# j04n-f/Encrypt-zkVM

Measured on AMD Instinct MI355X. Metric: STARK prove: trace-steps/sec at 2^20 steps; achieved HBM GB/s vs 8 TB/s peak, higher is better.
Workload: dtype f128

## Files before the change

encrypt-zkvm_amd/csrc/diag.hip:

```cpp
#include <hip/hip_runtime.h>
#include <string.h>

#include <algorithm>
#include <mutex>
#include <string>
#include <vector>

#include "blake3.hpp"
#include "host_pool.hpp"
#include "prover_internal.hpp"

using namespace zk;

namespace zk {
__global__ void k_field_op(int op, const fe *a, const fe *b, fe *out, size_t count, const fe_ws *ws, const fe_w2 *w2) {
    size_t t = blockIdx.x * (size_t)blockDim.x + threadIdx.x;
    if (t >= count) return;
    fe x = a[t], y = b[t];
    fe r;
    const size_t w0 = t & ~(size_t)63, mir = count - 1 - t;
    switch (op) {
    case 11: r = fe_mul_uniform(x, load_fe_ws(ws, (int)w0)); break;
    case 12: r = fe_mul_wsv(x, ws[t]); break;
    case 13: {
// ... 762 lines not shown
    for (int k = 0; k < W; k++) {
        TS.mode[k] = modes[k];
        if (modes[k] == CoeffSrc::ZERO) TS.plane[k] = nullptr;
        if (modes[k] != CoeffSrc::PLAIN) TS.lagr = p->polys + (size_t)W * n;
    }
    const Planes b = planes(p, ext);
    return with_kx(ext, [&](auto kx) -> int {
        constexpr int KX = decltype(kx)::value;
        typedef Chal<KX> X;
        const typename X::T zz = X::make(zv), zzg = X::make(zgv);
        ood_eval(p->st, TS, W, p->cpolys, ccols, log_n, zz, zzg, b.ood_tab, b.partials, p->ood);
        std::vector<fe> raw((size_t)KX * ood_out_values(TS, W, ccols)), hv((size_t)KX * (2 * W + ccols));
        ZK_TRY(p.down(raw.data(), p->ood, raw.size()));
        ood_fold_sources(KX, W, ccols, TS, wv, raw.data(), hv.data());
        memcpy(ood_out, hv.data(), hv.size() * sizeof(fe));
        DeepConsts<KX> D;
        memset(&D, 0, sizeof D);
        for (int k = 0; k < W; k++) D.alpha_t[k] = X::make(at[k]);
        for (int k = 0; k < C; k++) D.alpha_c[k] = X::make(ac[k]);
        D.z = zz, D.zg = zzg;
        deep_source_weight(D, TS, wv);
        ZK_CHECK_HIP(hipMemcpy(b.deep_consts, &D, sizeof D, hipMemcpyHostToDevice));
        const fe *Dk = deep_poly(p->st, TS, p->cpolys, C, log_n, b.deep_consts, zz, zzg, b.dscratch);
        ZK_TRY(p.down(deep_out, Dk, (size_t)KX * n));
        ZK_CHECK_HIP(hipMemsetAsync(p->flag, 0, 4, p->st));
        ZK_CHECK_HIP(hipMemsetAsync(p->ctmp, 0, (size_t)KX * n * 16, p->st));
        for (int j = 0; j < KX; j++)
            boundary_poly_add(p->st, TS, wv, log_n, K[j], cv, p->dscratch, p->ctmp + (size_t)j * n, p->flag);
        ZK_TRY(p.down(col0_out, p->ctmp, (size_t)KX * n));
        return p.down(flag_out, p->flag, 1);
    });
}

extern "C" int zk_diag_fri_layer(int device, const uint8_t *layer, size_t L, int ext, int fold, int lb, size_t wstride,
                                 const uint8_t *alpha, uint8_t *root_out, uint8_t *next_out) {
    fe2 av;
    const size_t N = L * wstride;
    const bool ok = layer && alpha && root_out && next_out && (ext == 1 || ext == 2) &&
                    (fold == 2 || fold == 4 || fold == 8 || fold == 16) && L && !(L & (L - 1)) && wstride &&
                    !(wstride & (wstride - 1)) && (L >= 4 * (size_t)fold || L == (size_t)fold) && N >= 128 &&
                    N <= ((size_t)1 << 22) && lb >= 0 && ((size_t)1 << lb) <= L / fold;
    if (!ok || !diag_read_fe(alpha, ext, &av))
        ZK_FAIL(ZK_ERR_INVALID_ARG, "zk_diag_fri_layer: L and wstride powers of two, 128 <= L wstride <= 2^22, fold 2 .. 16, "
                                    "at least 4 rows or the single row of an overfolded last layer, 2^lb <= L / fold, "
                                    "alpha canonical");
    DiagProver p;
    ZK_TRY(p.open(device, N / 8, 8, true, ext));
    const Planes b = planes(p, ext);
    const size_t rows = L / fold;
    uint8_t *leaves = p->fri_dig, *nodes = leaves + 32 * rows;
    ZK_CHECK_HIP(hipMemsetAsync(leaves, 0xA5, 64 * rows + 64, p->st));
    ZK_TRY(p.up(b.deep, layer, (size_t)ext * L));
    ZK_TRY(with_kx(ext, [&](auto kx) -> int {
        const auto F = fold_consts<decltype(kx)::value>(av, (uint32_t)fold);
        ZK_CHECK_HIP(hipMemcpy(b.fold_consts, &F, sizeof F, hipMemcpyHostToDevice));
        return ZK_OK;
    }));
    commit_fri_layer(p->st, ext, b.deep, L, fold, leaves, nodes, lb);
    fri_fold_launch(p->st, ext, b.deep, L, fold, b.fold_consts, p.pl->TN, wstride, b.fri, lb);
    ZK_TRY(p.down(root_out, nodes + 32, 32));
    return p.down(next_out, b.fri, (size_t)ext * rows);
}

constexpr size_t ZK_DIAG_MERKLE_GUARD = 4096;
extern "C" int zk_diag_merkle(int device, const uint8_t *leaves, size_t nl, int l3_min_log, uint32_t pf_blocks,
                              uint32_t block_p, uint8_t *nodes_out, uint8_t *guard_out, uint8_t *leaves_out,
                              const uint64_t *positions, size_t k, uint8_t *proof_out, size_t *proof_len) {
    if (!leaves || !nodes_out || !guard_out || !leaves_out || nl < 2 || (nl & (nl - 1)) || nl > ((size_t)1 << 24))
        ZK_FAIL(ZK_ERR_INVALID_ARG, "zk_diag_merkle: nl a power of two in [2, 2^24]");
    if (l3_min_log < 2 || l3_min_log > 62 || pf_blocks < 1 || pf_blocks > (1u << 20) || block_p < 1 || block_p > 512 ||
        (block_p & (block_p - 1)))
        ZK_FAIL(ZK_ERR_INVALID_ARG, "zk_diag_merkle: l3_min_log in [2, 62], pf_blocks in [1, 2^20], block_p a power of two "
                                    "in [1, 512]");
    if (positions && !proof_len) ZK_FAIL(ZK_ERR_INVALID_ARG, "zk_diag_merkle: positions without proof_len");
    std::vector<uint64_t> pos;
    if (positions) ZK_TRY(query_positions(positions, k, nl, pos));
    const size_t G = ZK_DIAG_MERKLE_GUARD, heap = 32 * nl;
    DiagBuf buf;
    ZK_TRY(buf.alloc(device, 2 * G + 2 * heap));
    uint8_t *d_nodes = buf.d + G, *d_leaves = buf.d + 2 * G + heap;
    ZK_CHECK_HIP(hipMemset(buf.d, 0xA5, 2 * G + heap));
    ZK_CHECK_HIP(hipMemcpy(d_leaves, leaves, heap, hipMemcpyHostToDevice));
    merkle_tree_cfg(nullptr, d_leaves, nl, d_nodes, MerkleCfg{l3_min_log, pf_blocks, block_p});
    ZK_CHECK_HIP(hipGetLastError());
    ZK_CHECK_HIP(hipMemcpy(nodes_out, d_nodes, heap, hipMemcpyDeviceToHost));
    ZK_CHECK_HIP(hipMemcpy(guard_out, buf.d, G, hipMemcpyDeviceToHost));
    ZK_CHECK_HIP(hipMemcpy(guard_out + G, d_nodes + heap, G, hipMemcpyDeviceToHost));
    ZK_CHECK_HIP(hipMemcpy(leaves_out, d_leaves, heap, hipMemcpyDeviceToHost));
    if (positions) ZK_TRY(batch_proof_bytes(nl, pos, d_leaves, d_nodes, proof_out, proof_len));
    return ZK_OK;
}

constexpr size_t ZK_DIAG_CE_GUARD = 4096;
extern "C" int zk_diag_ce_layout(int device, const uint8_t *in, size_t n, int ext, int to_natural, uint32_t max_blocks,
// ... 186 lines not shown
```

encrypt-zkvm_amd/csrc/fri_small.hpp:

```cpp
#pragma once
#include "f128.hpp"

namespace zk {
template <int F>
__device__ __forceinline__ void idft_small(fe v[F], const fe *zinv) {
    constexpr int LOGF = F == 2 ? 1 : F == 4 ? 2 : F == 8 ? 3 : 4;
    fe w[F];
#pragma unroll
    for (int k = 0; k < F; k++) {
        int r = 0;
#pragma unroll
        for (int b = 0; b < LOGF; b++) r |= ((k >> b) & 1) << (LOGF - 1 - b);
        w[r] = v[k];
    }
#pragma unroll
    for (int len = 2; len <= F; len <<= 1) {
#pragma unroll
        for (int start = 0; start < F; start += len) {
#pragma unroll
            for (int j = 0; j < len / 2; j++) {
                const fe u = w[start + j];
                const fe t = j == 0 ? w[start + j + len / 2] : fe_mul(w[start + j + len / 2], zinv[j * (F / len)]);
                w[start + j] = fe_add(u, t);
                w[start + j + len / 2] = fe_sub(u, t);
            }
        }
    }
#pragma unroll
    for (int k = 0; k < F; k++) v[k] = w[k];
}

}
```

encrypt-zkvm_amd/csrc/kernels.hip:

```cpp
#include <hip/hip_runtime.h>
#include <bitset>
#include <mutex>
#include <stdlib.h>
#include <string.h>

#include "blake3.hpp"
#include "fri_small.hpp"
#include "rescue_consts.hpp"
#include "zk_internal.hpp"

namespace zk {

#define ZK_LAUNCH_CHECK() (void)hipGetLastError()

__device__ __forceinline__ fe ld_fe(const fe *p) { return *p; }
__device__ __forceinline__ void st_fe(fe *p, fe v) { *p = v; }

template <class T>
__device__ __forceinline__ T pow_split(const T *lo, const T *hi, size_t t) {
    return ChalOf<T>::mul(lo[t & 2047], hi[t >> 11]);
}

#ifndef ZK_NTT_THREADS
#define ZK_NTT_THREADS 1024
#endif
#ifndef ZK_NTT_TILE
#define ZK_NTT_TILE 4096
#endif
#ifndef ZK_NTT_WAVES
#define ZK_NTT_WAVES 8
#endif
constexpr int NTT_THREADS = ZK_NTT_THREADS;

#ifndef ZK_NTT_LAZY
#define ZK_NTT_LAZY 1
#endif
#ifndef ZK_NTT_J0
#define ZK_NTT_J0 1
#endif
#ifndef ZK_NTT_SWZ
// ... 995 lines not shown
        v[0] = w.x;
        v[1] = w.y;
        v[2] = w.z;
        v[3] = w.w;
    }
#pragma unroll
    for (int e = 0; e < 4; e++) {
        const size_t i = i0 + e;
        out[i] = i == n - 1 ? nc.last[k] : fe{(uint64_t)v[e], 0};
    }
}

void expand_narrow(hipStream_t st, const uint8_t *src, const NarrowCols &nc, size_t n, fe *trace) {
    if (!nc.count) return;
    hipLaunchKernelGGL(k_expand_narrow, dim3(cdiv(n / 4, 256), nc.count), dim3(256), 0, st, src, nc, n, trace);
}

void commit_rows_coset_major(hipStream_t st, const fe *base, int ncols, int log_n, int log_b, uint8_t *leaves,
                             uint8_t *nodes) {
    const size_t N = (size_t)1 << (log_n + log_b);
    hash_rows_cosets(st, base, ncols, log_n, log_b, 0, log_b, leaves);
    merkle_tree(st, leaves, N, nodes);
}

__device__ __forceinline__ size_t fri_at(FriLayout f, size_t i) {
    return ((i & (((size_t)1 << f.lb) - 1)) << f.lcn) + (i >> f.lb);
}
FriLayout fri_layout(size_t L, int lb) {
    int lg = 0;
    while (((size_t)1 << lg) < L) lg++;
    return FriLayout{lb, lg - lb};
}

template <int KX>
__global__ void __launch_bounds__(256) k_hash_fri_rows(const fe *layer, size_t L, int fold, FriLayout f, uint8_t *leaves) {
    const size_t rows = L / fold;
    for (size_t r = blockIdx.x * (size_t)blockDim.x + threadIdx.x; r < rows; r += (size_t)gridDim.x * blockDim.x) {
        uint32_t h[8];
        b3::hash_elements(KX * fold, [&](int t) { return layer[(size_t)(t % KX) * L + fri_at(f, r + (size_t)(t / KX) * rows)]; }, h);
        store_digest(leaves + 32 * r, h);
    }
}

void commit_fri_layer(hipStream_t st, int KX, const fe *layer, size_t L, int fold, uint8_t *leaves, uint8_t *nodes, int lb) {
    const size_t rows = L / fold;
    const FriLayout f = fri_layout(L, lb);
    const dim3 grid(cdiv(rows, 256));
    if (KX == 1)
        ZK_PROF(st, "hash_fri_rows", 16.0 * L + 32.0 * rows, hipLaunchKernelGGL(k_hash_fri_rows<1>, grid, dim3(256), 0, st, layer, L, fold, f, leaves));
    else
        ZK_PROF(st, "hash_fri_rows_ext", 32.0 * L + 32.0 * rows, hipLaunchKernelGGL(k_hash_fri_rows<2>, grid, dim3(256), 0, st, layer, L, fold, f, leaves));
    if (rows == 1) (void)hipMemsetAsync(nodes + 32, 0, 32, st);
    merkle_tree(st, leaves, rows, nodes);
}

constexpr unsigned MERKLE_PF_BLOCKS = 2048;
__device__ __forceinline__ void merge_half3(const uint4 c[8], uint8_t *nodes, size_t cnt, size_t t, int half,
                                            uint32_t g[8]) {
    uint32_t l[8], r[8], h0[8], h1[8];
    auto dig = [&](int k, uint32_t d[8]) {
        const uint4 a = c[2 * k], b = c[2 * k + 1];
        d[0] = a.x; d[1] = a.y; d[2] = a.z; d[3] = a.w;
        d[4] = b.x; d[5] = b.y; d[6] = b.z; d[7] = b.w;
    };
    const size_t c0 = 4 * t + 2 * half;
    dig(0, l);
    dig(1, r);
    b3::merge(l, r, h0);
    store_digest(nodes + 32 * (cnt + c0), h0);
    dig(2, l);
    dig(3, r);
    b3::merge(l, r, h1);
    store_digest(nodes + 32 * (cnt + c0 + 1), h1);
    b3::merge(h0, h1, g);
    store_digest(nodes + 32 * (cnt / 2 + 2 * t + half), g);
}
#ifndef ZK_MERKLE_WAVES
#define ZK_MERKLE_WAVES 4
#endif
__global__ void __launch_bounds__(256, ZK_MERKLE_WAVES) k_merge_level3_pf(const uint8_t *src, uint8_t *nodes, size_t cnt) {
    const size_t q = cnt / 4, stride = (size_t)gridDim.x * blockDim.x;
    size_t t = blockIdx.x * (size_t)blockDim.x + threadIdx.x;
    const uint4 *s4 = reinterpret_cast<const uint4 *>(src);
    uint4 cur[8], nxt[8];
// ... 766 lines not shown

__global__ void __launch_bounds__(256) k_poly_degrees(const fe *polys, size_t len, DegReport *rep) {
    __shared__ unsigned long long sh_top[4];
    const int k = blockIdx.y;
    const fe *c = polys + (size_t)k * len;
    unsigned long long top = 0;
    for (size_t j = blockIdx.x * (size_t)blockDim.x + threadIdx.x; j < len; j += (size_t)gridDim.x * blockDim.x)
        if (!fe_is_zero(c[j])) top = j + 1;
    for (int d = 32; d > 0; d >>= 1) {
        const unsigned long long o = __shfl_xor(top, d, 64);
        top = o > top ? o : top;
    }
    if ((threadIdx.x & 63) == 0) sh_top[threadIdx.x >> 6] = top;
    __syncthreads();
    if (threadIdx.x == 0) {
        for (int w = 1; w < 4; w++) top = sh_top[w] > top ? sh_top[w] : top;
        if (top) {
            atomicMax(&rep->top[k], top - 1);
            atomicOr(&rep->nonzero, 1u << k);
        }
    }
}

void poly_degrees(hipStream_t st, const fe *polys, size_t len, int count, DegReport *rep) {
    unsigned blocks = cdiv(len, 256);
    if (blocks > 1024) blocks = 1024;
    ZK_PROF(st, "poly_degrees", 16.0 * count * (double)len,
            hipLaunchKernelGGL(k_poly_degrees, dim3(blocks, count), dim3(256), 0, st, polys, len, rep));
}

struct CrossWs {
    fe_ws w1, w2, w3, inv3n, k7[7];
};
__global__ void __launch_bounds__(256) k_comp_cross(CrossMap m, const fe *wi_lo, const fe *wi_hi,
                                                    const fe *i3_lo, const fe *i3_hi, fe scale, CrossWs cw,
                                                    int ncols, fe *polys, unsigned *nonzero) {
    for (size_t kl = blockIdx.x * (size_t)blockDim.x + threadIdx.x; kl < m.kcount; kl += (size_t)gridDim.x * blockDim.x) {
        const size_t k1 = m.k0 + kl;
        fe w = pow_split(wi_lo, wi_hi, k1);
        fe d[8];
        fe wr = fe_one();
#pragma unroll
        for (int r = 0; r < 8; r++) {
            if (r == 7 && m.derive7) {
                acc192 a7 = acc192_zero();
#pragma unroll
                for (int j = 0; j < 7; j++) acc192_madd_uniform(a7, d[j], cw.k7[j]);
                d[7] = acc192_reduce(a7);
                break;
            }
            fe v = m.c[r][kl];
            d[r] = r ? fe_mul(v, wr) : v;
            wr = fe_mul(wr, w);
        }
        fe e0 = d[0], e1 = d[4], e2 = d[2], e3 = d[6], e4 = d[1], e5 = d[5], e6 = d[3], e7 = d[7];
        fe t0 = fe_add(e0, e1), t1 = fe_sub(e0, e1), t2 = fe_add(e2, e3), t3 = fe_sub(e2, e3);
        fe t4 = fe_add(e4, e5), t5 = fe_sub(e4, e5), t6 = fe_add(e6, e7), t7 = fe_sub(e6, e7);
        t3 = fe_mul_uniform(t3, cw.w2);
        t7 = fe_mul_uniform(t7, cw.w2);
        fe u0 = fe_add(t0, t2), u2 = fe_sub(t0, t2), u1 = fe_add(t1, t3), u3 = fe_sub(t1, t3);
        fe u4 = fe_add(t4, t6), u6 = fe_sub(t4, t6), u5 = fe_add(t5, t7), u7 = fe_sub(t5, t7);
        u5 = fe_mul_uniform(u5, cw.w1);
        u6 = fe_mul_uniform(u6, cw.w2);
        u7 = fe_mul_uniform(u7, cw.w3);
        fe bk[8] = {fe_add(u0, u4), fe_add(u1, u5), fe_add(u2, u6), fe_add(u3, u7),
                    fe_sub(u0, u4), fe_sub(u1, u5), fe_sub(u2, u6), fe_sub(u3, u7)};
        fe s = fe_mul(scale, pow_split(i3_lo, i3_hi, k1));
        unsigned nz = 0;
#pragma unroll
        for (int k2 = 0; k2 < 8; k2++) {
            fe a = fe_mul(bk[k2], s);
            if (k2 < ncols) polys[(size_t)k2 * m.pstride + kl] = a;
            else nz |= !fe_is_zero(a);
            s = fe_mul_uniform(s, cw.inv3n);
        }
        if (nz) atomicOr(nonzero, 1u);
    }
}

void comp_cross_mapped(hipStream_t st, const CrossMap &m, const NttTables &T8n, const PowTable &inv3, fe scale,
                       fe w8inv, fe inv3n, int ncols, fe *polys, unsigned *nonzero_flag) {
    unsigned blocks = cdiv(m.kcount, 256);
    if (blocks > 65536) blocks = 65536;
    CrossWs cw;
    const fe w2 = fe_mul(w8inv, w8inv);
    cw.w1 = make_fe_ws(w8inv), cw.w2 = make_fe_ws(w2), cw.w3 = make_fe_ws(fe_mul(w2, w8inv));
    cw.inv3n = make_fe_ws(inv3n);
    for (int j = 0; j < 7; j++) cw.k7[j] = make_fe_ws(m.k7[j]);
    ZK_PROF(st, "comp_cross", (128.0 + 16.0 * ncols) * m.kcount, hipLaunchKernelGGL(k_comp_cross, dim3(blocks), dim3(256), 0, st, m, T8n.inv_lo,
                                                 T8n.inv_hi, inv3.lo, inv3.hi, scale, cw, ncols, polys,
                                                 nonzero_flag));
}

template <bool COEFFS>
__global__ void __launch_bounds__(256) k_cross_degrees(DegCrossMap m, const fe *wi_lo, const fe *wi_hi,
                                                       const fe *i3_lo, const fe *i3_hi, fe scale, CrossWs cw,
                                                       DegReport *rep) {
    __shared__ unsigned long long sh_top[4];
    const int k = blockIdx.y;
    const fe *c = m.c + (size_t)k * m.cstride;
    unsigned long long top = 0;
    for (size_t kl = blockIdx.x * (size_t)blockDim.x + threadIdx.x; kl < m.kcount; kl += (size_t)gridDim.x * blockDim.x) {
        const size_t k1 = m.k0 + kl;
        fe w = pow_split(wi_lo, wi_hi, k1);
        fe d[8];
        fe wr = fe_one();
#pragma unroll
        for (int r = 0; r < 8; r++) {
            fe v = c[m.off[r] + kl];
            d[r] = r ? fe_mul(v, wr) : v;
            wr = fe_mul(wr, w);
        }
        fe e0 = d[0], e1 = d[4], e2 = d[2], e3 = d[6], e4 = d[1], e5 = d[5], e6 = d[3], e7 = d[7];
        fe t0 = fe_add(e0, e1), t1 = fe_sub(e0, e1), t2 = fe_add(e2, e3), t3 = fe_sub(e2, e3);
        fe t4 = fe_add(e4, e5), t5 = fe_sub(e4, e5), t6 = fe_add(e6, e7), t7 = fe_sub(e6, e7);
        t3 = fe_mul_uniform(t3, cw.w2);
        t7 = fe_mul_uniform(t7, cw.w2);
        fe u0 = fe_add(t0, t2), u2 = fe_sub(t0, t2), u1 = fe_add(t1, t3), u3 = fe_sub(t1, t3);
        fe u4 = fe_add(t4, t6), u6 = fe_sub(t4, t6), u5 = fe_add(t5, t7), u7 = fe_sub(t5, t7);
        u5 = fe_mul_uniform(u5, cw.w1);
// ... 55 lines not shown
        ZK_PROF(st, "cross_degrees", 128.0 * m.count * (double)m.kcount,
                hipLaunchKernelGGL(k_cross_degrees<false>, grid, dim3(256), 0, st, m, T8n.inv_lo, T8n.inv_hi, inv3.lo,
                                   inv3.hi, scale, cw, rep));
}

constexpr int OOD_GROUP = 7;

template <int KX>
__global__ void k_ood_tables(typename Chal<KX>::T z, typename Chal<KX>::T zg, uint64_t chunk, int nw,
                             typename Chal<KX>::T *tab) {
    typedef typename Chal<KX>::T T;
    const int t = blockIdx.x * blockDim.x + threadIdx.x;
    if (t >= 128 + 2 * nw) return;
    T x;
    uint64_t e;
    if (t < 128) {
        x = t < 64 ? z : zg;
        e = t & 63;
    } else {
        const int u = t - 128;
        x = u < nw ? z : zg;
        e = chunk * (uint64_t)(u < nw ? u : u - nw);
    }
    tab[t] = Chal<KX>::exp(x, e);
}

struct OodPolys {
    static constexpr int MAXP = CoeffSrc::MAXC + 16 + 1;
    int count, count2;
    uint32_t zero;
    const fe *poly[MAXP];
    uint8_t rz[MAXP], rg[MAXP];
};
template <int KX, int E>
__global__ void __launch_bounds__(256) k_ood_eval(OodPolys L, int W, int np, size_t n, const typename Chal<KX>::T *tab,
                                                  int nw, int w0, int w1, fe *partials) {
    typedef Chal<KX> X;
    typedef typename X::T T;
    const int gw = w0 + (int)((blockIdx.x * blockDim.x + threadIdx.x) >> 6);
    const int lane = threadIdx.x & 63;
    const size_t plane = (size_t)np * nw;
    const int tg = (L.count2 + OOD_GROUP - 1) / OOD_GROUP, g = blockIdx.y;
    const bool two = g < tg;
    const int p0 = two ? g * OOD_GROUP : L.count2 + (g - tg) * OOD_GROUP;
    const int p1 = min(two ? L.count2 : L.count, p0 + OOD_GROUP);
    const size_t base = (size_t)gw * 64 * E + lane;
    __shared__ T Y[2][E];
    if (threadIdx.x < 2 * E) {
        const int which = threadIdx.x / E, e = threadIdx.x % E;
        const T y = which ? X::mul(tab[127], tab[65]) : X::mul(tab[63], tab[1]);
        Y[which][e] = X::exp(y, (uint64_t)e);
    }
    __syncthreads();
    if (gw >= w1) return;
    if (blockIdx.y == 0 && L.zero && lane == 0)
        for (int c = 0; c < W; c++)
            if ((L.zero >> c) & 1u) {
                X::st(partials + (size_t)c * nw + gw, plane, X::zero());
                X::st(partials + (size_t)(W + c) * nw + gw, plane, X::zero());
            }
    const T wz = X::mul(tab[lane], tab[128 + gw]);
    const T wzg = two ? X::mul(tab[64 + lane], tab[128 + nw + gw]) : X::zero();
    for (int p = p0; p < p1; p++) {
        const fe *c = L.poly[p] + base;
        fe v[E];
#pragma unroll
        for (int e = 0; e < E; e++) v[e] = base + 64 * (size_t)e < n ? c[64 * e] : fe_zero();
        const T hz = wave_sum(X::mul(dot_base<E>(v, Y[0]), wz));
        if (lane == 0) X::st(partials + (size_t)L.rz[p] * nw + gw, plane, hz);
        if (two) {
            const T hg = wave_sum(X::mul(dot_base<E>(v, Y[1]), wzg));
            if (lane == 0) X::st(partials + (size_t)L.rg[p] * nw + gw, plane, hg);
        }
    }
}

int ood_waves(size_t n) { return (int)std::max<size_t>(1, n / 1024); }

template <class T>
void ood_eval(hipStream_t st, const CoeffSrc &S, int W, const fe *cpolys, int C, int log_n, T z, T zg, fe *tab,
              fe *partials, fe *out, int rank, int G) {
    constexpr int KX = ChalOf<T>::KX;
    const size_t n = (size_t)1 << log_n;
    const int E = n >= 1024 ? 16 : std::max<int>(1, (int)(n / 64));
    const int nw = (int)((n + 64 * E - 1) / (64 * E));
    const int w0 = (int)((int64_t)nw * rank / G), w1 = (int)((int64_t)nw * (rank + 1) / G);
    T *t = reinterpret_cast<T *>(tab);
    hipLaunchKernelGGL(k_ood_tables<KX>, dim3(cdiv(128 + 2 * nw, 256)), dim3(256), 0, st, z, zg, (uint64_t)64 * E, nw, t);
    const int np = ood_out_values(S, W, C);
    OodPolys L{};
    auto add = [&L](const fe *poly, int rz, int rg) {
        L.poly[L.count] = poly, L.rz[L.count] = (uint8_t)rz, L.rg[L.count] = (uint8_t)rg;
        L.count++;
    };
    for (int c = 0; c < W; c++) {
        if (S.mode[c] == CoeffSrc::ZERO) L.zero |= 1u << c;
        else add(S.plane[c], c, W + c);
    }
    if (S.lagr) add(S.lagr, np - 2, np - 1);
    L.count2 = L.count;
    for (int j = 0; j < C; j++) add(cpolys + (size_t)j * n, 2 * W + j, 0);
    const dim3 grid(std::max(1u, cdiv(w1 - w0, 4)),
                    (L.count2 + OOD_GROUP - 1) / OOD_GROUP + (L.count - L.count2 + OOD_GROUP - 1) / OOD_GROUP);
    const char *name = KX == 1 ? "ood_eval" : "ood_eval_ext";
// ... 274 lines not shown
}
template <class T>
const fe *deep_poly(hipStream_t st, const CoeffSrc &TS, const fe *cpolys, int ccols, int log_n,
                    const void *deep_consts_dev, T z, T zg, fe *scratch) {
    const size_t n = (size_t)1 << log_n;
    deep_tables(st, n, z, zg, scratch);
    deep_phase1<T>(st, TS, cpolys, ccols, n, deep_consts_dev, scratch, 0, n, nullptr);
    deep_phase3(st, n, z, zg, scratch, 0, n, nullptr);
    return DeepScratch(scratch, n, ChalOf<T>::KX).out;
}
template <class T>
const fe *deep_range_begin(hipStream_t st, const CoeffSrc &TS, const fe *cpolys, int ccols, int log_n,
                           const void *deep_consts_dev, T z, T zg, fe *scratch, size_t k0, size_t kn) {
    const size_t n = (size_t)1 << log_n;
    deep_tables(st, n, z, zg, scratch);
    fe *total = DeepScratch(scratch, n, ChalOf<T>::KX).total;
    deep_phase1<T>(st, TS, cpolys, ccols, n, deep_consts_dev, scratch, k0, kn, total);
    return total;
}
template <class T>
const fe *deep_range_end(hipStream_t st, int log_n, T z, T zg, fe *scratch, size_t k0, size_t kn, const fe *ext) {
    const size_t n = (size_t)1 << log_n;
    deep_phase3(st, n, z, zg, scratch, k0, kn, ext);
    return DeepScratch(scratch, n, ChalOf<T>::KX).out;
}

struct BndPoly {
    static constexpr int MAXT = 13;
    int nt;
    fe bnd1;
    const fe *plane[MAXT];
    fe c0[MAXT], c1[MAXT];
};
__global__ void __launch_bounds__(DIV_T) k_bnd_div_g(BndPoly bp, const fe *pw, size_t H, fe *g1, fe *g2, fe *bs,
                                                    size_t kbase, size_t kend) {
    __shared__ fe red[DIV_T / 64];
    const size_t per = 2048 + H;
    const size_t k = kbase + blockIdx.x * (size_t)DIV_T + threadIdx.x;
    fe v1 = fe_zero(), v2 = fe_zero();
    if (k < kend) {
        acc288 a0 = acc288_zero(), a1 = acc288_zero();
        for (int i = 0; i < bp.nt; i++) {
            const fe t = ld_fe(bp.plane[i] + k);
            acc288_madd(a0, bp.c0[i], t);
            acc288_madd(a1, bp.c1[i], t);
        }
        v1 = acc288_reduce(a0);
        fe f1 = acc288_reduce(a1);
        if (k == 0) f1 = fe_sub(f1, bp.bnd1);
        v2 = fe_mul(f1, pow_split(pw + per, pw + per + 2048, k));
        g1[k] = v1;
        g2[k] = v2;
    }
    v1 = block_sum256(v1, red);
    v2 = block_sum256(v2, red);
    if (threadIdx.x == 0) {
        bs[2 * blockIdx.x] = v1;
        bs[2 * blockIdx.x + 1] = v2;
    }
}

static void bnd_tables_phase1(hipStream_t st, const CoeffSrc &TS, const fe *w, size_t n, const AirConsts &K, fe c,
                              fe *scratch, size_t k0, size_t kn, fe *total) {
    const DeepScratch S(scratch, n, 1);
    const size_t nb1 = (kn + DIV_T - 1) / DIV_T;
    DeepPowBases<1> pb;
    pb.b[0] = fe_one();
    pb.b[1] = c;
    pb.b[2] = fe_one();
    pb.b[3] = fe_inv(c);
    hipLaunchKernelGGL(k_deep_pow_tables<1>, dim3(cdiv(4 * (2048 + S.H), 256)), dim3(256), 0, st, pb, S.H, S.pw);
    BndPoly bp{};
    bp.bnd1 = K.bnd1;
    static const int col0[12] = {0, 7, 8, 11, 12, 13, 14, 15, 16, 17, 18, 19};
    fe le0 = fe_zero(), le1 = fe_zero();
    for (int i = 0; i < 12; i++) {
        const int cc = col0[i];
        const fe b0 = K.coeff_b[i], b1 = i == 0 || i == 3 ? fe_zero() : K.coeff_b[i < 3 ? 11 + i : 10 + i];
// ... 71 lines not shown

__device__ __forceinline__ bool fe_canon_dev(uint32_t w0, uint32_t w1, uint32_t w2, uint32_t w3) {
    const uint64_t lo = (uint64_t)w0 | ((uint64_t)w1 << 32), hi = (uint64_t)w2 | ((uint64_t)w3 << 32);
    return !(hi == ZK_P_HI && lo >= ZK_P_LO);
}
__global__ void k_fri_coin(uint32_t *seed, const uint8_t *root, int k, fe *alpha_out, fe *alpha_log) {
    if (threadIdx.x != 0 || blockIdx.x != 0) return;
    uint32_t s[8], r[8], h[8];
    for (int i = 0; i < 8; i++) s[i] = seed[i];
    load_digest(root, r);
    b3::merge(s, r, h);
    for (int i = 0; i < 8; i++) seed[i] = h[i];
    for (uint32_t ctr = 1; ctr < 1000; ctr++) {
        uint32_t m[16] = {h[0], h[1], h[2], h[3], h[4], h[5], h[6], h[7], ctr, 0, 0, 0, 0, 0, 0, 0};
        uint32_t d[8];
        b3::iv(d);
        b3::compress(d, m, 0, 0, 40, b3::CHUNK_START | b3::CHUNK_END | b3::ROOT);
        if (fe_canon_dev(d[0], d[1], d[2], d[3]) && (k == 1 || fe_canon_dev(d[4], d[5], d[6], d[7]))) {
            const fe a0 = fe{(uint64_t)d[0] | ((uint64_t)d[1] << 32), (uint64_t)d[2] | ((uint64_t)d[3] << 32)};
            const fe a1 = fe{(uint64_t)d[4] | ((uint64_t)d[5] << 32), (uint64_t)d[6] | ((uint64_t)d[7] << 32)};
            alpha_out[0] = alpha_log[0] = a0;
            if (k == 2) alpha_out[1] = alpha_log[1] = a1;
            return;
        }
    }
}

void fri_coin_launch(hipStream_t st, uint32_t *seed_dev, const uint8_t *root_dev, int k, fe *alpha_dev,
                     fe *alpha_log) {
    hipLaunchKernelGGL(k_fri_coin, dim3(1), dim3(64), 0, st, seed_dev, root_dev, k, alpha_dev, alpha_log);
}


template <int KX, int F>
__global__ void __launch_bounds__(256) k_fri_fold(const fe *layer, size_t L, const FoldConsts<KX> *Fc, const fe *wi_lo,
                                                  const fe *wi_hi, size_t wstride, FriLayout f, fe *next) {
    typedef Chal<KX> X;
    typedef typename X::T T;
    const size_t rows = L / F;
    for (size_t r = blockIdx.x * (size_t)blockDim.x + threadIdx.x; r < rows; r += (size_t)gridDim.x * blockDim.x) {
        fe va[F], vb[KX == 2 ? F : 1];
#pragma unroll
        for (int k = 0; k < F; k++) {
            const size_t at = fri_at(f, r + (size_t)k * rows);
            va[k] = layer[at];
            if constexpr (KX == 2) vb[k] = layer[L + at];
        }
        const T beta = X::mulb(Fc->alpha, fe_mul(Fc->inv_offset, pow_split(wi_lo, wi_hi, r * wstride)));
        idft_small<F>(va, Fc->zinv);
        if constexpr (KX == 2) idft_small<F>(vb, Fc->zinv);
        auto V = [&](int m) -> T {
            if constexpr (KX == 2) return fe2{va[m], vb[m]};
            else return va[m];
        };
        T acc = V(F - 1);
#pragma unroll
        for (int m = F - 2; m >= 0; m--) acc = X::add(X::mul(acc, beta), V(m));
        X::st(next + r, rows, X::mulb(acc, Fc->inv_fold));
    }
}

template <int KX>
static void fri_fold_kx(hipStream_t st, const fe *layer, size_t L, int fold, const void *fold_consts_dev,
                        const NttTables &TN, size_t wstride, fe *next, int lb) {
    unsigned blocks = cdiv(L / fold, 256);
    if (blocks > 65536) blocks = 65536;
    const FoldConsts<KX> *F = (const FoldConsts<KX> *)fold_consts_dev;
    const FriLayout fl = fri_layout(L, lb);
    const char *name = KX == 1 ? "fri_fold" : "fri_fold_ext";
#define ZK_FOLD(FF) ZK_PROF(st, name, KX * (16.0 * L + 16.0 * (L / fold)), hipLaunchKernelGGL((k_fri_fold<KX, FF>), dim3(blocks), dim3(256), 0, st, layer, L, F, TN.inv_lo, TN.inv_hi, wstride, fl, next))
    switch (fold) {
        case 2: ZK_FOLD(2); break;
        case 4: ZK_FOLD(4); break;
        case 8: ZK_FOLD(8); break;
        default: ZK_FOLD(16); break;
    }
#undef ZK_FOLD
}
void fri_fold_launch(hipStream_t st, int KX, const fe *layer, size_t L, int fold, const void *fold_consts_dev,
                     const NttTables &TN, size_t wstride, fe *next, int lb) {
    if (KX == 1) fri_fold_kx<1>(st, layer, L, fold, fold_consts_dev, TN, wstride, next, lb);
    else fri_fold_kx<2>(st, layer, L, fold, fold_consts_dev, TN, wstride, next, lb);
}

__global__ void k_gather_chunks(const uint64_t *addr, size_t k, fe *out) {
    const size_t t = blockIdx.x * (size_t)blockDim.x + threadIdx.x;
    if (t < k) out[t] = *reinterpret_cast<const fe *>((uintptr_t)addr[t]);
}

__global__ void __launch_bounds__(256) k_copy_to_host(CopyList L) {
    const int e = blockIdx.y;
    if (e >= L.n) return;
    const uint32_t *src = L.src[e];
    uint32_t *dst = L.dst[e];
    for (size_t w = blockIdx.x * (size_t)blockDim.x + threadIdx.x; w < L.words[e]; w += (size_t)gridDim.x * blockDim.x)
        dst[w] = src[w];
    __threadfence_system();
}

hipError_t copy_to_host(hipStream_t st, const CopyList &L, size_t max_words) {
    if (L.n <= 0) return hipSuccess;
    const unsigned bx = std::max(1u, std::min(cdiv(max_words, 256), 64u));
    hipLaunchKernelGGL(k_copy_to_host, dim3(bx, (unsigned)L.n), dim3(256), 0, st, L);
    return hipGetLastError();
}

void gather_chunks(hipStream_t st, const uint64_t *addr, size_t k, fe *out) {
    if (k) ZK_PROF(st, "gather_chunks", 24.0 * k, hipLaunchKernelGGL(k_gather_chunks, dim3(cdiv(k, 256)), dim3(256), 0, st, addr, k, out));
}

__global__ void k_gather_fe(const fe *src, const uint64_t *idx, size_t k, fe *out) {
    size_t t = blockIdx.x * (size_t)blockDim.x + threadIdx.x;
    if (t < k) out[t] = src[idx[t]];
}

// ... 112 lines not shown
```

encrypt-zkvm_amd/csrc/zk_internal.hpp:

```cpp
#pragma once
#include <hip/hip_runtime.h>
#include <stddef.h>
#include <stdint.h>

#include <string>
#include <vector>

#include "chal.hpp"
#include "f128.hpp"

namespace zk {

static inline unsigned cdiv(size_t a, size_t b) { return (unsigned)((a + b - 1) / b); }

struct KernelProfiler {
    bool on = false;
    struct Rec {
        const char *name;
        hipEvent_t a, b;
        double bytes;
        double muls, addsubs;
    };
    std::vector<Rec> recs;
    std::vector<hipEvent_t> pool;
// ... 284 lines not shown
    DeepScratch(fe *s, size_t n, int KX)
        : H(n / 2048 + 2),
          pw(s),
          g1(pw + 4 * KX * (2048 + H)),
          g2(g1 + KX * n),
          out(g2 + KX * n),
          bs(out + KX * n),
          total(bs + 2 * KX * ((n + ZK_DEEP_BLOCK - 1) / ZK_DEEP_BLOCK)) {}
    static size_t size(size_t n, int KX) { return KX * (4 * (2048 + n / 2048 + 2) + 3 * n + 2 * (n / ZK_DEEP_BLOCK + 1)); }
};
template <class T>
const fe *deep_poly(hipStream_t st, const CoeffSrc &S, const fe *cpolys, int ccols, int log_n,
                    const void *deep_consts_dev, T z, T zg, fe *scratch);
constexpr size_t ZK_DEEP_RANGE_QUANTUM = 2048;
template <class T>
const fe *deep_range_begin(hipStream_t st, const CoeffSrc &S, const fe *cpolys, int ccols, int log_n,
                           const void *deep_consts_dev, T z, T zg, fe *scratch, size_t k0, size_t kn);
template <class T>
const fe *deep_range_end(hipStream_t st, int log_n, T z, T zg, fe *scratch, size_t k0, size_t kn, const fe *ext);
template <class T>
void deep_coeff_launch(hipStream_t st, const NttTables &Tn, const CoeffSrc &S, const fe *cpolys, int ccols, int log_n,
                       int log_b, const void *deep_consts_dev, T z, T zg, const CosetTables &CT, fe *scratch,
                       fe *ulde, fe *ntt_tmp, fe *out);
template <int KX>
struct FoldConsts {
    fe zinv[16];
    typename Chal<KX>::T alpha;
    fe inv_offset, inv_fold;
};
static_assert(sizeof(FoldConsts<1>) == 19 * sizeof(fe) && offsetof(FoldConsts<1>, alpha) == 16 * sizeof(fe) &&
                  offsetof(FoldConsts<2>, alpha) == 16 * sizeof(fe),
              "FoldConsts layout");
void commit_fri_layer(hipStream_t st, int KX, const fe *layer, size_t L, int fold, uint8_t *leaves, uint8_t *nodes,
                      int lb = 0);
void fri_fold_launch(hipStream_t st, int KX, const fe *layer, size_t L, int fold, const void *fold_consts_dev,
                     const NttTables &TN, size_t wstride, fe *next, int lb = 0);
void coset_major_to_natural(hipStream_t st, const fe *src, int log_n, int log_b, fe *dst);
constexpr unsigned ZK_CE_LAYOUT_BLOCKS = 2048;
void ce_layout(hipStream_t st, const fe *src, size_t n, int ext, bool to_natural, fe *dst, unsigned max_blocks = 0);
constexpr unsigned ZK_ROWS_LAYOUT_BLOCKS = 1280;
void rows_layout(hipStream_t st, const fe *base, int ncols, size_t n, int log_b, size_t first, size_t count, fe *dst,
                 unsigned max_blocks = 0);
void interleave_columns(hipStream_t st, const fe *src, size_t n, int ncols, fe *dst);
void fri_coin_launch(hipStream_t st, uint32_t *seed_dev, const uint8_t *root_dev, int k, fe *alpha_dev,
                     fe *alpha_log);

void gather_fe(hipStream_t st, const fe *src, const uint64_t *idx, size_t k, fe *out);

}
```

Measured before the change: 124.8 million.

## Specialize FRI hashing/fold per fold, precompute twiddle constants, batch loads in several kernels

The FRI row-hash kernel is templated on the fold factor and now does explicit unrolled BLAKE3 compression. The fold kernel uses host-precomputed fe_ws twiddles and inverse constants with uniform multiplies. comp_cross folds the scale into the per-row twiddle chain and replaces the running inv3n power with precomputed powers. It also gets a launch-bounds occupancy hint. ood_eval software-pipelines coefficient loads in two halves and caches twiddle products in shared memory, and boundary division batches plane loads. A capped-block diagnostic entry point is also added. These changes cut redundant multiplies and expose load-level parallelism, at the cost of more template instances and register pressure.

```diff
diff --git a/encrypt-zkvm_amd/csrc/diag.hip b/encrypt-zkvm_amd/csrc/diag.hip
--- a/encrypt-zkvm_amd/csrc/diag.hip
+++ b/encrypt-zkvm_amd/csrc/diag.hip
@@ -818,18 +818,18 @@
     });
 }
 
-extern "C" int zk_diag_fri_layer(int device, const uint8_t *layer, size_t L, int ext, int fold, int lb, size_t wstride,
-                                 const uint8_t *alpha, uint8_t *root_out, uint8_t *next_out) {
+static int diag_fri_layer(int device, const uint8_t *layer, size_t L, int ext, int fold, int lb, size_t wstride,
+                          const uint8_t *alpha, uint32_t max_blocks, uint8_t *root_out, uint8_t *next_out) {
     fe2 av;
     const size_t N = L * wstride;
     const bool ok = layer && alpha && root_out && next_out && (ext == 1 || ext == 2) &&
                     (fold == 2 || fold == 4 || fold == 8 || fold == 16) && L && !(L & (L - 1)) && wstride &&
                     !(wstride & (wstride - 1)) && (L >= 4 * (size_t)fold || L == (size_t)fold) && N >= 128 &&
-                    N <= ((size_t)1 << 22) && lb >= 0 && ((size_t)1 << lb) <= L / fold;
+                    N <= ((size_t)1 << 22) && lb >= 0 && ((size_t)1 << lb) <= L / fold && max_blocks <= (1u << 20);
     if (!ok || !diag_read_fe(alpha, ext, &av))
         ZK_FAIL(ZK_ERR_INVALID_ARG, "zk_diag_fri_layer: L and wstride powers of two, 128 <= L wstride <= 2^22, fold 2 .. 16, "
                                     "at least 4 rows or the single row of an overfolded last layer, 2^lb <= L / fold, "
-                                    "alpha canonical");
+                                    "alpha canonical, max_blocks at most 2^20");
     DiagProver p;
     ZK_TRY(p.open(device, N / 8, 8, true, ext));
     const Planes b = planes(p, ext);
@@ -842,10 +842,19 @@
         ZK_CHECK_HIP(hipMemcpy(b.fold_consts, &F, sizeof F, hipMemcpyHostToDevice));
         return ZK_OK;
     }));
-    commit_fri_layer(p->st, ext, b.deep, L, fold, leaves, nodes, lb);
-    fri_fold_launch(p->st, ext, b.deep, L, fold, b.fold_consts, p.pl->TN, wstride, b.fri, lb);
+    commit_fri_layer(p->st, ext, b.deep, L, fold, leaves, nodes, lb, max_blocks);
+    fri_fold_launch(p->st, ext, b.deep, L, fold, b.fold_consts, p.pl->TN, wstride, b.fri, lb, max_blocks);
     ZK_TRY(p.down(root_out, nodes + 32, 32));
     return p.down(next_out, b.fri, (size_t)ext * rows);
+}
+extern "C" int zk_diag_fri_layer(int device, const uint8_t *layer, size_t L, int ext, int fold, int lb, size_t wstride,
+                                 const uint8_t *alpha, uint8_t *root_out, uint8_t *next_out) {
+    return diag_fri_layer(device, layer, L, ext, fold, lb, wstride, alpha, 0, root_out, next_out);
+}
+extern "C" int zk_diag_fri_layer_capped(int device, const uint8_t *layer, size_t L, int ext, int fold, int lb,
+                                        size_t wstride, const uint8_t *alpha, uint32_t max_blocks, uint8_t *root_out,
+                                        uint8_t *next_out) {
+    return diag_fri_layer(device, layer, L, ext, fold, lb, wstride, alpha, max_blocks, root_out, next_out);
 }
 
 constexpr size_t ZK_DIAG_MERKLE_GUARD = 4096;
diff --git a/encrypt-zkvm_amd/csrc/fri_small.hpp b/encrypt-zkvm_amd/csrc/fri_small.hpp
--- a/encrypt-zkvm_amd/csrc/fri_small.hpp
+++ b/encrypt-zkvm_amd/csrc/fri_small.hpp
@@ -30,4 +30,32 @@
     for (int k = 0; k < F; k++) v[k] = w[k];
 }
 
+template <int F>
+__device__ __forceinline__ void idft_small_ws(fe v[F], const fe_ws *zw) {
+    constexpr int LOGF = F == 2 ? 1 : F == 4 ? 2 : F == 8 ? 3 : 4;
+    fe w[F];
+#pragma unroll
+    for (int k = 0; k < F; k++) {
+        int r = 0;
+#pragma unroll
+        for (int b = 0; b < LOGF; b++) r |= ((k >> b) & 1) << (LOGF - 1 - b);
+        w[r] = v[k];
+    }
+#pragma unroll
+    for (int len = 2; len <= F; len <<= 1) {
+#pragma unroll
+        for (int start = 0; start < F; start += len) {
+#pragma unroll
+            for (int j = 0; j < len / 2; j++) {
+                const fe u = w[start + j];
+                const fe t = j == 0 ? w[start + j + len / 2] : fe_mul_uniform(w[start + j + len / 2], zw[j * (F / len) - 1]);
+                w[start + j] = fe_add(u, t);
+                w[start + j + len / 2] = fe_sub(u, t);
+            }
+        }
+    }
+#pragma unroll
+    for (int k = 0; k < F; k++) v[k] = w[k];
 }
+
+}
diff --git a/encrypt-zkvm_amd/csrc/kernels.hip b/encrypt-zkvm_amd/csrc/kernels.hip
--- a/encrypt-zkvm_amd/csrc/kernels.hip
+++ b/encrypt-zkvm_amd/csrc/kernels.hip
@@ -6,6 +6,7 @@
 
 #include "blake3.hpp"
 #include "fri_small.hpp"
+#include "host_field.hpp"
 #include "rescue_consts.hpp"
 #include "zk_internal.hpp"
 
@@ -1067,24 +1068,62 @@
     return FriLayout{lb, lg - lb};
 }
 
-template <int KX>
-__global__ void __launch_bounds__(256) k_hash_fri_rows(const fe *layer, size_t L, int fold, FriLayout f, uint8_t *leaves) {
-    const size_t rows = L / fold;
+template <int KX, int F>
+__global__ void __launch_bounds__(256) k_hash_fri_rows(const fe *layer, size_t L, FriLayout f, uint8_t *leaves) {
+    constexpr int NE = KX * F, CH = NE < 16 ? NE : 16;
+    const size_t rows = L / F;
     for (size_t r = blockIdx.x * (size_t)blockDim.x + threadIdx.x; r < rows; r += (size_t)gridDim.x * blockDim.x) {
         uint32_t h[8];
-        b3::hash_elements(KX * fold, [&](int t) { return layer[(size_t)(t % KX) * L + fri_at(f, r + (size_t)(t / KX) * rows)]; }, h);
+        b3::iv(h);
+#pragma unroll
+        for (int c0 = 0; c0 < NE; c0 += CH) {
+            fe v[CH];
+#pragma unroll
+            for (int t = 0; t < CH; t++)
+                v[t] = layer[(size_t)((c0 + t) % KX) * L + fri_at(f, r + (size_t)((c0 + t) / KX) * rows)];
+#pragma unroll
+            for (int b = 0; b < (CH + 3) / 4; b++) {
+                uint32_t m[16];
+#pragma unroll
+                for (int e = 0; e < 4; e++) {
+                    const fe x = 4 * b + e < CH ? v[4 * b + e] : fe_zero();
+                    m[4 * e + 0] = (uint32_t)x.lo, m[4 * e + 1] = (uint32_t)(x.lo >> 32);
+                    m[4 * e + 2] = (uint32_t)x.hi, m[4 * e + 3] = (uint32_t)(x.hi >> 32);
+                }
+                constexpr int NB = (NE + 3) / 4;
+                const int bi = c0 / 4 + b;
+                const uint32_t len = (uint32_t)(16 * NE - 64 * bi < 64 ? 16 * NE - 64 * bi : 64);
+                const uint32_t flags = (bi == 0 ? b3::CHUNK_START : 0) | (bi == NB - 1 ? (b3::CHUNK_END | b3::ROOT) : 0);
+                b3::compress(h, m, 0, 0, len, flags);
+            }
+        }
         store_digest(leaves + 32 * r, h);
     }
 }
 
-void commit_fri_layer(hipStream_t st, int KX, const fe *layer, size_t L, int fold, uint8_t *leaves, uint8_t *nodes, int lb) {
+template <int KX>
+static void hash_fri_rows_kx(hipStream_t st, const fe *layer, size_t L, int fold, FriLayout f, uint8_t *leaves,
+                             unsigned max_blocks) {
+    const size_t rows = L / fold;
+    unsigned blocks = cdiv(rows, 256);
+    if (max_blocks && blocks > max_blocks) blocks = max_blocks;
+    const char *name = KX == 1 ? "hash_fri_rows" : "hash_fri_rows_ext";
+#define ZK_HASH_FRI(FF) ZK_PROF(st, name, KX * 16.0 * L + 32.0 * rows, hipLaunchKernelGGL((k_hash_fri_rows<KX, FF>), dim3(blocks), dim3(256), 0, st, layer, L, f, leaves))
+    switch (fold) {
+        case 2: ZK_HASH_FRI(2); break;
+        case 4: ZK_HASH_FRI(4); break;
+        case 8: ZK_HASH_FRI(8); break;
+        default: ZK_HASH_FRI(16); break;
+    }
+#undef ZK_HASH_FRI
+}
+
+void commit_fri_layer(hipStream_t st, int KX, const fe *layer, size_t L, int fold, uint8_t *leaves, uint8_t *nodes, int lb,
+                      unsigned max_blocks) {
     const size_t rows = L / fold;
     const FriLayout f = fri_layout(L, lb);
-    const dim3 grid(cdiv(rows, 256));
-    if (KX == 1)
-        ZK_PROF(st, "hash_fri_rows", 16.0 * L + 32.0 * rows, hipLaunchKernelGGL(k_hash_fri_rows<1>, grid, dim3(256), 0, st, layer, L, fold, f, leaves));
-    else
-        ZK_PROF(st, "hash_fri_rows_ext", 32.0 * L + 32.0 * rows, hipLaunchKernelGGL(k_hash_fri_rows<2>, grid, dim3(256), 0, st, layer, L, fold, f, leaves));
+    if (KX == 1) hash_fri_rows_kx<1>(st, layer, L, fold, f, leaves, max_blocks);
+    else hash_fri_rows_kx<2>(st, layer, L, fold, f, leaves, max_blocks);
     if (rows == 1) (void)hipMemsetAsync(nodes + 32, 0, 32, st);
     merkle_tree(st, leaves, rows, nodes);
 }
@@ -1917,14 +1956,17 @@
 struct CrossWs {
     fe_ws w1, w2, w3, inv3n, k7[7];
 };
-__global__ void __launch_bounds__(256) k_comp_cross(CrossMap m, const fe *wi_lo, const fe *wi_hi,
-                                                    const fe *i3_lo, const fe *i3_hi, fe scale, CrossWs cw,
+struct CompWs {
+    fe_ws w1, w2, w3, k7[7], i3n[7];
+};
+__global__ void __launch_bounds__(256, 5) k_comp_cross(CrossMap m, const fe *wi_lo, const fe *wi_hi,
+                                                    const fe *i3_lo, const fe *i3_hi, fe scale, CompWs cw,
                                                     int ncols, fe *polys, unsigned *nonzero) {
     for (size_t kl = blockIdx.x * (size_t)blockDim.x + threadIdx.x; kl < m.kcount; kl += (size_t)gridDim.x * blockDim.x) {
         const size_t k1 = m.k0 + kl;
-        fe w = pow_split(wi_lo, wi_hi, k1);
+        const fe w = pow_split(wi_lo, wi_hi, k1);
+        fe t = fe_mul(scale, pow_split(i3_lo, i3_hi, k1));
         fe d[8];
-        fe wr = fe_one();
 #pragma unroll
         for (int r = 0; r < 8; r++) {
             if (r == 7 && m.derive7) {
@@ -1934,9 +1976,8 @@
                 d[7] = acc192_reduce(a7);
                 break;
             }
-            fe v = m.c[r][kl];
-            d[r] = r ? fe_mul(v, wr) : v;
-            wr = fe_mul(wr, w);
+            d[r] = fe_mul(m.c[r][kl], t);
+            if (r < 6 || (r == 6 && !m.derive7)) t = fe_mul(t, w);
         }
         fe e0 = d[0], e1 = d[4], e2 = d[2], e3 = d[6], e4 = d[1], e5 = d[5], e6 = d[3], e7 = d[7];
         fe t0 = fe_add(e0, e1), t1 = fe_sub(e0, e1), t2 = fe_add(e2, e3), t3 = fe_sub(e2, e3);
@@ -1950,14 +1991,12 @@
         u7 = fe_mul_uniform(u7, cw.w3);
         fe bk[8] = {fe_add(u0, u4), fe_add(u1, u5), fe_add(u2, u6), fe_add(u3, u7),
                     fe_sub(u0, u4), fe_sub(u1, u5), fe_sub(u2, u6), fe_sub(u3, u7)};
-        fe s = fe_mul(scale, pow_split(i3_lo, i3_hi, k1));
         unsigned nz = 0;
 #pragma unroll
         for (int k2 = 0; k2 < 8; k2++) {
-            fe a = fe_mul(bk[k2], s);
+            const fe a = k2 ? fe_mul_uniform(bk[k2], cw.i3n[k2 - 1]) : bk[0];
             if (k2 < ncols) polys[(size_t)k2 * m.pstride + kl] = a;
             else nz |= !fe_is_zero(a);
-            s = fe_mul_uniform(s, cw.inv3n);
         }
         if (nz) atomicOr(nonzero, 1u);
     }
@@ -1967,10 +2006,11 @@
                        fe w8inv, fe inv3n, int ncols, fe *polys, unsigned *nonzero_flag) {
     unsigned blocks = cdiv(m.kcount, 256);
     if (blocks > 65536) blocks = 65536;
-    CrossWs cw;
+    CompWs cw;
     const fe w2 = fe_mul(w8inv, w8inv);
     cw.w1 = make_fe_ws(w8inv), cw.w2 = make_fe_ws(w2), cw.w3 = make_fe_ws(fe_mul(w2, w8inv));
-    cw.inv3n = make_fe_ws(inv3n);
+    fe s = inv3n;
+    for (int j = 0; j < 7; j++, s = fe_mul(s, inv3n)) cw.i3n[j] = make_fe_ws(s);
     for (int j = 0; j < 7; j++) cw.k7[j] = make_fe_ws(m.k7[j]);
     ZK_PROF(st, "comp_cross", (128.0 + 16.0 * ncols) * m.kcount, hipLaunchKernelGGL(k_comp_cross, dim3(blocks), dim3(256), 0, st, m, T8n.inv_lo,
                                                  T8n.inv_hi, inv3.lo, inv3.hi, scale, cw, ncols, polys,
@@ -2092,8 +2132,22 @@
     const fe *poly[MAXP];
     uint8_t rz[MAXP], rg[MAXP];
 };
+template <int KX, int H>
+__device__ __forceinline__ void ood_half(typename Chal<KX>::Acc &az, typename Chal<KX>::Acc &ag, const fe *v,
+                                         const typename Chal<KX>::T *yz, const typename Chal<KX>::T *yg, bool two) {
+    if (two) {
+#pragma unroll
+        for (int e = 0; e < H; e++) {
+            Chal<KX>::madd(az, yz[e], v[e]);
+            Chal<KX>::madd(ag, yg[e], v[e]);
+        }
+    } else {
+#pragma unroll
+        for (int e = 0; e < H; e++) Chal<KX>::madd(az, yz[e], v[e]);
+    }
+}
 template <int KX, int E>
-__global__ void __launch_bounds__(256) k_ood_eval(OodPolys L, int W, int np, size_t n, const typename Chal<KX>::T *tab,
+__global__ void __launch_bounds__(256, KX == 1 ? 4 : 3) k_ood_eval(OodPolys L, int W, int np, size_t n, const typename Chal<KX>::T *tab,
                                                   int nw, int w0, int w1, fe *partials) {
     typedef Chal<KX> X;
     typedef typename X::T T;
@@ -2119,17 +2173,37 @@
                 X::st(partials + (size_t)c * nw + gw, plane, X::zero());
                 X::st(partials + (size_t)(W + c) * nw + gw, plane, X::zero());
             }
-    const T wz = X::mul(tab[lane], tab[128 + gw]);
-    const T wzg = two ? X::mul(tab[64 + lane], tab[128 + nw + gw]) : X::zero();
+    const bool inb = base < n;
+    const size_t off = inb ? base : 0;
+    __shared__ T WZ[2][256];
+    WZ[0][threadIdx.x] = inb ? X::mul(tab[lane], tab[128 + gw]) : X::zero();
+    WZ[1][threadIdx.x] = two && inb ? X::mul(tab[64 + lane], tab[128 + nw + gw]) : X::zero();
+    constexpr int H0 = (E + 1) / 2, H1 = E - H0;
+    fe va[H0], vb[H1 ? H1 : 1];
+    auto load_a = [&](int p) {
+        const fe *c = L.poly[p] + off;
+#pragma unroll
+        for (int e = 0; e < H0; e++) va[e] = c[64 * e];
+    };
+    auto load_b = [&](int p) {
+        const fe *c = L.poly[p] + off;
+#pragma unroll
+        for (int e = 0; e < H1; e++) vb[e] = c[64 * (H0 + e)];
+    };
+    load_a(p0);
+    load_b(p0);
     for (int p = p0; p < p1; p++) {
-        const fe *c = L.poly[p] + base;
-        fe v[E];
-#pragma unroll
-        for (int e = 0; e < E; e++) v[e] = base + 64 * (size_t)e < n ? c[64 * e] : fe_zero();
-        const T hz = wave_sum(X::mul(dot_base<E>(v, Y[0]), wz));
+        typename X::Acc az = X::acc_zero(), ag = X::acc_zero();
+        ood_half<KX, H0>(az, ag, va, Y[0], Y[1], two);
+        if (p + 1 < p1) load_a(p + 1);
+        if constexpr (H1 > 0) {
+            ood_half<KX, H1>(az, ag, vb, Y[0] + H0, Y[1] + H0, two);
+            if (p + 1 < p1) load_b(p + 1);
+        }
+        const T hz = wave_sum(X::mul(X::reduce(az), WZ[0][threadIdx.x]));
         if (lane == 0) X::st(partials + (size_t)L.rz[p] * nw + gw, plane, hz);
         if (two) {
-            const T hg = wave_sum(X::mul(dot_base<E>(v, Y[1]), wzg));
+            const T hg = wave_sum(X::mul(X::reduce(ag), WZ[1][threadIdx.x]));
             if (lane == 0) X::st(partials + (size_t)L.rg[p] * nw + gw, plane, hg);
         }
     }
@@ -2470,6 +2544,7 @@
     const fe *plane[MAXT];
     fe c0[MAXT], c1[MAXT];
 };
+constexpr int BND_BATCH = 6;
 __global__ void __launch_bounds__(DIV_T) k_bnd_div_g(BndPoly bp, const fe *pw, size_t H, fe *g1, fe *g2, fe *bs,
                                                     size_t kbase, size_t kend) {
     __shared__ fe red[DIV_T / 64];
@@ -2478,10 +2553,16 @@
     fe v1 = fe_zero(), v2 = fe_zero();
     if (k < kend) {
         acc288 a0 = acc288_zero(), a1 = acc288_zero();
-        for (int i = 0; i < bp.nt; i++) {
-            const fe t = ld_fe(bp.plane[i] + k);
-            acc288_madd(a0, bp.c0[i], t);
-            acc288_madd(a1, bp.c1[i], t);
+        for (int i0 = 0; i0 < bp.nt; i0 += BND_BATCH) {
+            fe t[BND_BATCH];
+#pragma unroll
+            for (int j = 0; j < BND_BATCH; j++) t[j] = ld_fe(bp.plane[min(i0 + j, bp.nt - 1)] + k);
+#pragma unroll
+            for (int j = 0; j < BND_BATCH; j++)
+                if (i0 + j < bp.nt) {
+                    acc288_madd(a0, bp.c0[i0 + j], t[j]);
+                    acc288_madd(a1, bp.c1[i0 + j], t[j]);
+                }
         }
         v1 = acc288_reduce(a0);
         fe f1 = acc288_reduce(a1);
@@ -2619,9 +2700,14 @@
 }
 
 
+template <int F>
+struct FoldWs {
+    fe_ws zw[F > 2 ? F / 2 - 1 : 1], inv_offset, inv_fold;
+};
 template <int KX, int F>
-__global__ void __launch_bounds__(256) k_fri_fold(const fe *layer, size_t L, const FoldConsts<KX> *Fc, const fe *wi_lo,
-                                                  const fe *wi_hi, size_t wstride, FriLayout f, fe *next) {
+__global__ void __launch_bounds__(256) k_fri_fold(const fe *layer, size_t L, const FoldConsts<KX> *Fc, FoldWs<F> fw,
+                                                  const fe *wi_lo, const fe *wi_hi, size_t wstride, FriLayout f,
+                                                  fe *next) {
     typedef Chal<KX> X;
     typedef typename X::T T;
     const size_t rows = L / F;
@@ -2633,9 +2719,14 @@
             va[k] = layer[at];
             if constexpr (KX == 2) vb[k] = layer[L + at];
         }
-        const T beta = X::mulb(Fc->alpha, fe_mul(Fc->inv_offset, pow_split(wi_lo, wi_hi, r * wstride)));
-        idft_small<F>(va, Fc->zinv);
-        if constexpr (KX == 2) idft_small<F>(vb, Fc->zinv);
+        const T beta = X::mulb(Fc->alpha, fe_mul_uniform(pow_split(wi_lo, wi_hi, r * wstride), fw.inv_offset));
+        if constexpr (KX == 2 && F == 16) {
+            idft_small<F>(va, Fc->zinv);
+            idft_small<F>(vb, Fc->zinv);
+        } else {
+            idft_small_ws<F>(va, fw.zw);
+            if constexpr (KX == 2) idft_small_ws<F>(vb, fw.zw);
+        }
         auto V = [&](int m) -> T {
             if constexpr (KX == 2) return fe2{va[m], vb[m]};
             else return va[m];
@@ -2643,19 +2734,41 @@
         T acc = V(F - 1);
 #pragma unroll
         for (int m = F - 2; m >= 0; m--) acc = X::add(X::mul(acc, beta), V(m));
-        X::st(next + r, rows, X::mulb(acc, Fc->inv_fold));
-    }
+        if constexpr (KX == 2) {
+            next[r] = fe_mul_uniform(acc.a, fw.inv_fold);
+            next[rows + r] = fe_mul_uniform(acc.b, fw.inv_fold);
+        } else {
+            next[r] = fe_mul_uniform(acc, fw.inv_fold);
+        }
+    }
+}
+
+template <int F>
+static const FoldWs<F> &fold_ws() {
+    static const FoldWs<F> W = [] {
+        FoldWs<F> w{};
+        int lg = 0;
+        while ((1 << lg) < F) lg++;
+        const fe zeta_inv = fe_inv(h_root_of_unity(lg));
+        fe z = zeta_inv;
+        for (int t = 1; t < F / 2; t++, z = fe_mul(z, zeta_inv)) w.zw[t - 1] = make_fe_ws(z);
+        w.inv_offset = make_fe_ws(fe_inv(fe_make(3)));
+        w.inv_fold = make_fe_ws(fe_inv(fe_make(F)));
+        return w;
+    }();
+    return W;
 }
 
 template <int KX>
 static void fri_fold_kx(hipStream_t st, const fe *layer, size_t L, int fold, const void *fold_consts_dev,
-                        const NttTables &TN, size_t wstride, fe *next, int lb) {
+                        const NttTables &TN, size_t wstride, fe *next, int lb, unsigned max_blocks) {
     unsigned blocks = cdiv(L / fold, 256);
-    if (blocks > 65536) blocks = 65536;
+    if (!max_blocks) max_blocks = 65536;
+    if (blocks > max_blocks) blocks = max_blocks;
     const FoldConsts<KX> *F = (const FoldConsts<KX> *)fold_consts_dev;
     const FriLayout fl = fri_layout(L, lb);
     const char *name = KX == 1 ? "fri_fold" : "fri_fold_ext";
-#define ZK_FOLD(FF) ZK_PROF(st, name, KX * (16.0 * L + 16.0 * (L / fold)), hipLaunchKernelGGL((k_fri_fold<KX, FF>), dim3(blocks), dim3(256), 0, st, layer, L, F, TN.inv_lo, TN.inv_hi, wstride, fl, next))
+#define ZK_FOLD(FF) ZK_PROF(st, name, KX * (16.0 * L + 16.0 * (L / fold)), hipLaunchKernelGGL((k_fri_fold<KX, FF>), dim3(blocks), dim3(256), 0, st, layer, L, F, fold_ws<FF>(), TN.inv_lo, TN.inv_hi, wstride, fl, next))
     switch (fold) {
         case 2: ZK_FOLD(2); break;
         case 4: ZK_FOLD(4); break;
@@ -2665,9 +2778,9 @@
 #undef ZK_FOLD
 }
 void fri_fold_launch(hipStream_t st, int KX, const fe *layer, size_t L, int fold, const void *fold_consts_dev,
-                     const NttTables &TN, size_t wstride, fe *next, int lb) {
-    if (KX == 1) fri_fold_kx<1>(st, layer, L, fold, fold_consts_dev, TN, wstride, next, lb);
-    else fri_fold_kx<2>(st, layer, L, fold, fold_consts_dev, TN, wstride, next, lb);
+                     const NttTables &TN, size_t wstride, fe *next, int lb, unsigned max_blocks) {
+    if (KX == 1) fri_fold_kx<1>(st, layer, L, fold, fold_consts_dev, TN, wstride, next, lb, max_blocks);
+    else fri_fold_kx<2>(st, layer, L, fold, fold_consts_dev, TN, wstride, next, lb, max_blocks);
 }
 
 __global__ void k_gather_chunks(const uint64_t *addr, size_t k, fe *out) {
diff --git a/encrypt-zkvm_amd/csrc/zk_internal.hpp b/encrypt-zkvm_amd/csrc/zk_internal.hpp
--- a/encrypt-zkvm_amd/csrc/zk_internal.hpp
+++ b/encrypt-zkvm_amd/csrc/zk_internal.hpp
@@ -340,9 +340,9 @@
                   offsetof(FoldConsts<2>, alpha) == 16 * sizeof(fe),
               "FoldConsts layout");
 void commit_fri_layer(hipStream_t st, int KX, const fe *layer, size_t L, int fold, uint8_t *leaves, uint8_t *nodes,
-                      int lb = 0);
+                      int lb = 0, unsigned max_blocks = 0);
 void fri_fold_launch(hipStream_t st, int KX, const fe *layer, size_t L, int fold, const void *fold_consts_dev,
-                     const NttTables &TN, size_t wstride, fe *next, int lb = 0);
+                     const NttTables &TN, size_t wstride, fe *next, int lb = 0, unsigned max_blocks = 0);
 void coset_major_to_natural(hipStream_t st, const fe *src, int log_n, int log_b, fe *dst);
 constexpr unsigned ZK_CE_LAYOUT_BLOCKS = 2048;
 void ce_layout(hipStream_t st, const fe *src, size_t n, int ext, bool to_natural, fe *dst, unsigned max_blocks = 0);
diff --git a/encrypt-zkvm_amd/zkvm_amd/back_diag.py b/encrypt-zkvm_amd/zkvm_amd/back_diag.py
--- /dev/null
+++ b/encrypt-zkvm_amd/zkvm_amd/back_diag.py
@@ -0,0 +1,26 @@
+from __future__ import annotations
+
+import ctypes as C
+
+from . import native
+
+SYMBOL = "zk_diag_fri_layer_capped"
+_bound = False
+
+
+def _fn():
+    global _bound
+    f = getattr(native.lib(), SYMBOL)
+    if not _bound:
+        vp, sz, u32, i32 = C.c_void_p, C.c_size_t, C.c_uint32, C.c_int
+        f.argtypes = [i32, vp, sz, i32, i32, i32, sz, vp, u32, vp, vp]
+        f.restype = i32
+        _bound = True
+    return f
+
+
+def fri_layer_capped(layer: bytes, L: int, ext: int, fold: int, lb: int, wstride: int, alpha: bytes, max_blocks: int,
+                     device: int = 0):
+    root, nxt = C.create_string_buffer(32), C.create_string_buffer(16 * ext * (L // fold))
+    rc = _fn()(device, layer, L, ext, fold, lb, wstride, alpha, max_blocks, root, nxt)
+    return rc, root.raw, nxt.raw
```

Result: no change. 124.9 million (median of 3 runs) (+0.1%).
